# mittinatten/freesasa

Measured on AMD Instinct MI355X. Metric: atoms/sec SASA (L&R 20 slices), higher is better.
Workload: dtype f64

## Files before the change

### freesasa_amd/csrc/engine_internal.h

```cpp
#ifndef FREESASA_AMD_ENGINE_INTERNAL_H
#define FREESASA_AMD_ENGINE_INTERNAL_H

#include <hip/hip_runtime.h>

#include <atomic>
#include <functional>
#include <mutex>
#include <stdint.h>
#include <stddef.h>
#include <stdio.h>
#include <string>
#include <thread>
#include <unistd.h>
#include <vector>

#include "../../include/freesasa_gpu.h"
#include "../../include/freesasa_ingest.h"
#include "sasa_kernels.h"
#include "lr2_kernels.h"
#include "group_kernels.h"
#include "select_kernels.h"
#include "traj_kernels.h"
#include "xtc_kernels.h"
#include "pbc_kernels.h"
#include "pbc_tri_kernels.h"
#include "vol_kernels.h"
#include "dots_kernels.h"
#include "iface_kernels.h"
#include "contact_kernels.h"
#include "rescontact_kernels.h"
#include "ifsweep_kernels.h"
#include "gpu_parse.h"


#define SORT_B 1024
#define SORT_APT 16
#define SORT_ATOMS (SORT_B * SORT_APT - 256)
#define SORT_CELLS (1 << 18)
#define SORT_WORDS (SORT_CELLS / 32)
#define SORT_CELL_BITS 26

hipError_t kl_prep_fused(const sasa::PipeArgs &pa, hipStream_t st);
hipError_t kl_prep_general(const sasa::PipeArgs &pa, long long cells_cap, hipStream_t st);
hipError_t kl_lr2_main(int rmax, int grid, size_t lds, hipStream_t st, const sasa::Lr2Args &la);
hipError_t kl_lr2_mid(int grid, size_t lds, hipStream_t st, const sasa::Lr2Args &la);
hipError_t kl_lr_tile(int tier, const sasa::TileCfg &c, const sasa::TileArgs &t, int grid, size_t lds, hipStream_t st, bool bucket);
hipError_t kl_sr_tile(int tier, const sasa::TileCfg &c, const sasa::TileArgs &t, int grid, size_t lds, hipStream_t st, double *evec = nullptr, unsigned *masks = nullptr);
hipError_t kl_totals(const sasa::PipeArgs &pa, int n_chunks, int n_structs, const double *d_sasa, double *bpart, double *d_totals, hipStream_t st);
hipError_t kl_segment_sums(const double *d_sasa, const int64_t *d_seg, int n_segs, bool short_segments, double *d_out, hipStream_t st);
hipError_t kl_class_sums(const double *d_sasa, const unsigned char *d_class, const int64_t *d_offsets, int n_structs, double *d_out, hipStream_t st);
hipError_t kl_residue_areas(const double *d_sasa, const unsigned char *d_class, const unsigned char *d_backbone, const int64_t *d_res_first,
                            const short *d_ref_row, const double *d_ref_table, double *d_abs, double *d_rel, int n_res, hipStream_t st);
hipError_t kl_arc_kat(const double *d_arcs, const int *d_first, int n_sets, double *d_out, hipStream_t st);
hipError_t kl_widen_f32(const float *d_in, double *d_out, long long n, hipStream_t st);
hipError_t kl_narrow_f64(const double *d_in, float *d_out, long long n, hipStream_t st);
void kl_dump_phase_clocks(void);
hipError_t kl_grp_count(const sasa::GrpArgs &a, hipStream_t st);
hipError_t kl_grp_rank(const sasa::GrpArgs &a, hipStream_t st);
hipError_t kl_grp_finish(const sasa::GrpArgs &a, hipStream_t st);
hipError_t kl_grp_totals(const sasa::GrpArgs &a, hipStream_t st);
hipError_t kl_gid_struct(const sasa::GidArgs &a, hipStream_t st);
hipError_t kl_gid_label(const sasa::GidLabelArgs &a, hipStream_t st);

hipError_t kl_sel_mask(const sasa::SelArgs &a, hipStream_t st);
hipError_t kl_sel_sums(const sasa::SelArgs &a, hipStream_t st);

hipError_t kl_traj_gather(const sasa::TrajArgs &a, const void *d_in, bool in_f32, double *d_out, hipStream_t st);
hipError_t kl_traj_gather_dcd(const sasa::TrajDcdArgs &a, const void *d_in, bool big_endian, double *d_out, hipStream_t st);
hipError_t kl_traj_gather_nc(const sasa::TrajNcArgs &a, const void *d_in, double *d_out, hipStream_t st);
hipError_t kl_traj_gather_trr(const sasa::TrajTrrArgs &a, const void *d_in, bool is_double, double *d_out, hipStream_t st);
hipError_t kl_xtc_scan(const sasa::XtcArgs &a, hipStream_t st);
hipError_t kl_xtc_unpack(const sasa::XtcArgs &a, hipStream_t st);
hipError_t kl_traj_residues(const sasa::TrajArgs &a, hipStream_t st);
hipError_t kl_traj_class(const sasa::TrajArgs &a, hipStream_t st);
hipError_t kl_traj_sel(const sasa::TrajArgs &a, hipStream_t st);
hipError_t kl_traj_group_radii(const sasa::TrajGroupArgs &a, hipStream_t st);
hipError_t kl_traj_group_gather(const sasa::TrajGroupArgs &a, hipStream_t st);
hipError_t kl_traj_group_finish(const sasa::TrajGroupArgs &a, hipStream_t st);
hipError_t kl_traj_group_totals(const sasa::TrajGroupArgs &a, hipStream_t st);
hipError_t kl_traj_stats(const sasa::TrajStatsArgs &a, hipStream_t st);

hipError_t kl_pbc_count(const sasa::PbcArgs &a, hipStream_t st);
hipError_t kl_pbc_emit(const sasa::PbcArgs &a, hipStream_t st);
hipError_t kl_pbc_collect(const sasa::PbcArgs &a, hipStream_t st);
hipError_t kl_pbc_tri_count(const sasa::PbcTriArgs &a, hipStream_t st);
hipError_t kl_pbc_tri_emit(const sasa::PbcTriArgs &a, hipStream_t st);
hipError_t kl_gpbc_cells(const sasa::GpbcArgs &a, hipStream_t st);
hipError_t kl_gpbc_finish(const sasa::GpbcArgs &a, hipStream_t st);

hipError_t kl_vol_origin(const sasa::VolArgs &a, hipStream_t st);
hipError_t kl_vol_atom(const sasa::VolArgs &a, hipStream_t st);

hipError_t kl_dots_count(const sasa::DotsArgs &a, hipStream_t st);
hipError_t kl_dots_expand(const sasa::DotsArgs &a, hipStream_t st);

hipError_t kl_iface_box(const sasa::IfaceArgs &a, hipStream_t st);
hipError_t kl_iface_candidates(const sasa::IfaceArgs &a, hipStream_t st);
hipError_t kl_iface_contact(const sasa::IfaceArgs &a, hipStream_t st);
hipError_t kl_iface_gather(const sasa::IfaceArgs &a, hipStream_t st);
hipError_t kl_iface_finish(const sasa::IfaceArgs &a, hipStream_t st);
hipError_t kl_iface_res_scan(int *a, int64_t n, int *scratch, hipStream_t st);
hipError_t kl_iface_res_segments(const sasa::IfaceResArgs &a, int *scratch, hipStream_t st);
hipError_t kl_iface_res_rows(const sasa::IfaceResArgs &a, int *scratch, hipStream_t st);
hipError_t kl_contact_masks(const sasa::ContactArgs &a, hipStream_t st);
hipError_t kl_contact_attribute(const sasa::ContactArgs &a, hipStream_t st);
hipError_t kl_contact_rows(const sasa::ContactArgs &a, int *scratch, hipStream_t st);
hipError_t kl_rc_segments(const sasa::IfaceResArgs &s, int *scratch, hipStream_t st);
hipError_t kl_rc_fold(const sasa::ResContactArgs &a, int *scratch, hipStream_t st);
hipError_t kl_ifs_side_class(const sasa::IfsClassArgs &a, hipStream_t st);
hipError_t kl_ifs_res_rows(const sasa::IfsRowArgs &a, hipStream_t st);


struct DevBuf {
    void *p = nullptr;
    size_t cap = 0;
};

struct freesasa_gpu_ctx {
    int device = 0;
    hipStream_t stream = nullptr;
    bool own_stream = false;
    bool timing = false;
    bool shared_radii = false;
    char err[512] = {0};
    freesasa_gpu_stats stats = {};
// ... 433 lines not shown
```

### freesasa_amd/csrc/gpu_engine.hip

```cpp
#include <hip/hip_runtime.h>

#include <math.h>
#include <atomic>
#include <new>
#include <stdarg.h>
#include <stdint.h>
#include <stdio.h>
#include <stdlib.h>
#include <string.h>
#include <vector>

#include "engine_internal.h"

using namespace sasa;


int ctx_fail(freesasa_gpu_ctx *c, const char *fmt, ...)
{
    va_list ap;
    va_start(ap, fmt);
    vsnprintf(c->err, sizeof c->err, fmt, ap);
    va_end(ap);
    return -1;
}
// ... 345 lines not shown
{
    c->err[0] = 0;
    if (deferred) *deferred = false;
    if (!d_xyz || !d_radii || !offsets || !d_sasa) return ctx_fail(c, "null argument");
    if (n_structs <= 0) return ctx_fail(c, "n_structs must be > 0");
    if (resolution <= 0) return ctx_fail(c, "resolution must be > 0");
    if (offsets[0] != 0) return ctx_fail(c, "offsets[0] must be 0");
    for (int s = 0; s < n_structs; ++s)
        if (offsets[s + 1] < offsets[s]) return ctx_fail(c, "offsets must be non-decreasing");
    const int64_t n64 = offsets[n_structs];
    if (n64 <= 0) return ctx_fail(c, "empty batch");
    if (n64 > (int64_t)1 << 30) return ctx_fail(c, "batch too large (max 2^30 atoms per call)");
    const int n = (int)n64;

    HIP_TRY(c, hipSetDevice(c->device));
    hipStream_t st = c->stream;
    const size_t nb = (size_t)n;

    if (ensure(c, c->offsets, sizeof(int64_t) * ((size_t)n_structs + 1)) || ensure(c, c->grid, sizeof(GridS) * (size_t)n_structs) ||
        ensure(c, c->ncells, sizeof(long long) * ((size_t)n_structs + 1)) || ensure(c, c->sid, 4 * nb) ||
        ensure(c, c->cell_of, 8 * nb) || ensure(c, c->rank, 4 * nb) || ensure(c, c->sq, 32 * nb) ||
        ensure(c, c->s_idx, 16 * nb) ||
        ensure(c, c->status, sizeof(int) * ST_WORDS))
        return -1;

    if ((int)c->offsets_host.size() != n_structs + 1 ||
        memcmp(c->offsets_host.data(), offsets, sizeof(int64_t) * ((size_t)n_structs + 1)) != 0) {
        if (c->pend[0].active || c->pend[1].active) HIP_TRY(c, hipStreamSynchronize(st));
        c->offsets_host.clear();
        std::vector<int> cs, cl, sc0((size_t)n_structs + 1);
        std::vector<int64_t> cb;
        for (int s = 0; s < n_structs; ++s) {
            sc0[s] = (int)cs.size();
            for (int64_t b = offsets[s]; b < offsets[s + 1]; b += SASA_BOUNDS_CHUNK) {
                const int64_t e = b + SASA_BOUNDS_CHUNK < offsets[s + 1] ? b + SASA_BOUNDS_CHUNK : offsets[s + 1];
                cs.push_back(s); cb.push_back(b); cl.push_back((int)(e - b));
            }
        }
        sc0[n_structs] = (int)cs.size();
        c->n_chunks = (int)cs.size();
        const size_t nc = cs.size();
        if (ensure(c, c->chunk_struct, 4 * nc) || ensure(c, c->chunk_begin, 8 * nc) || ensure(c, c->chunk_len, 4 * nc) ||
            ensure(c, c->struct_chunk0, 4 * ((size_t)n_structs + 1)) || ensure(c, c->bpart, 56 * nc))
            return -1;
        HIP_TRY(c, hipMemcpy(c->offsets.p, offsets, sizeof(int64_t) * ((size_t)n_structs + 1), hipMemcpyHostToDevice));
        HIP_TRY(c, hipMemcpy(c->chunk_struct.p, cs.data(), 4 * nc, hipMemcpyHostToDevice));
        HIP_TRY(c, hipMemcpy(c->chunk_begin.p, cb.data(), 8 * nc, hipMemcpyHostToDevice));
        HIP_TRY(c, hipMemcpy(c->chunk_len.p, cl.data(), 4 * nc, hipMemcpyHostToDevice));
        HIP_TRY(c, hipMemcpy(c->struct_chunk0.p, sc0.data(), 4 * ((size_t)n_structs + 1), hipMemcpyHostToDevice));
        c->offsets_host.assign(offsets, offsets + n_structs + 1);
    }
    HIP_TRY(c, hipMemsetAsync(c->status.p, 0, (sizeof(int) * ST_WORDS + 63) & ~(size_t)63, st));
    if (c->timing) HIP_TRY(c, hipEventRecord(ctx_ev(c)[0], st));

    PipeArgs pa;
    memset(&pa, 0, sizeof pa);
    pa.xyz = d_xyz; pa.radii = d_radii; pa.offsets = (const int64_t *)c->offsets.p;
    pa.n_structs = n_structs; pa.n_atoms = n; pa.probe = probe; pa.max_cells = c->max_cells;
    pa.shared_radii = c->shared_radii ? 1 : 0;
    pa.n_chunks = c->n_chunks; pa.chunk_struct = (const int *)c->chunk_struct.p; pa.chunk_begin = (const int64_t *)c->chunk_begin.p;
    pa.chunk_len = (const int *)c->chunk_len.p; pa.struct_chunk0 = (const int *)c->struct_chunk0.p; pa.bpart = (double *)c->bpart.p;
    pa.grid = (GridS *)c->grid.p; pa.ncells = (long long *)c->ncells.p;
    pa.sid = (int *)c->sid.p; pa.cell_of = (long long *)c->cell_of.p; pa.rank = (int *)c->rank.p;
    pa.sq = (Quad *)c->sq.p;
    pa.s_idx = (SortIdx *)c->s_idx.p;
    pa.status = (int *)c->status.p;
    pa.cells_total = (long long *)((int *)c->status.p + ST_CELLS);
    pa.cells_total_at = pa.cells_total - pa.ncells;
    if (probe != c->hint_probe) {
        c->hint_res[0] = c->hint_res[1] = 0;
        c->hint_pool2 = 0;
        c->hint_probe = probe;
    }
    pa.occ_stride = c->hint_res[lr ? 0 : 1] == resolution ? 0 : (n / 256 > 0 ? n / 256 : 1);

    int *status_h = ctx_status_h(c);
    long long cells_cap = 10LL * n + 256LL * n_structs;
    if (cells_cap < c->cells_hint) cells_cap = c->cells_hint;
    if (cells_cap > c->max_cells) cells_cap = c->max_cells;
    const int nblk_scan = (int)((cells_cap + 1 + (long long)SASA_PIPE_B * SASA_SCAN_ITEMS - 1) / ((long long)SASA_PIPE_B * SASA_SCAN_ITEMS));
    long long biggest = 0;
    for (int s_ = 0; s_ < n_structs; ++s_) biggest = offsets[s_ + 1] - offsets[s_] > biggest ? offsets[s_ + 1] - offsets[s_] : biggest;
    static const long long small_fused = getenv("FREESASA_AMD_SMALL_FUSED") ? atoll(getenv("FREESASA_AMD_SMALL_FUSED")) : 4096;
    const bool fused = c->sort_fused && biggest <= SORT_ATOMS && (n_structs >= 8 || biggest <= small_fused) && !getenv("FREESASA_AMD_NO_FUSED_SORT");
    const bool compact = fused && (!lr || (lr2_supported(resolution) && !getenv("FREESASA_AMD_LR1"))) && !getenv("FREESASA_AMD_DENSE_CELLS");
    if (compact) {
        if (ensure(c, c->cell_tbl, sizeof(unsigned long long) * ((size_t)(cells_cap >> 5) + 2)) || ensure(c, c->cell_first, sizeof(int) * (nb + (size_t)n_structs + 2)))
            return -1;
        pa.cell_tbl = (unsigned long long *)c->cell_tbl.p;
        pa.cell_first = (int *)c->cell_first.p;
    } else {
        const size_t desc_cap_was = c->blk_sums.cap;
        if (ensure(c, c->cell_start, sizeof(int) * ((size_t)cells_cap + 4)) || ensure(c, c->blk_sums, sizeof(unsigned long long) * ((size_t)nblk_scan + 1)))
            return -1;
        if (c->blk_sums.cap != desc_cap_was) HIP_TRY(c, hipMemsetAsync(c->blk_sums.p, 0, c->blk_sums.cap, st));
    }
    pa.cell_start = (int *)c->cell_start.p;
    pa.scan_desc = (unsigned long long *)c->blk_sums.p;
    c->scan_epoch = c->scan_epoch >= (1 << 30) - 1 ? 1 : c->scan_epoch + 1;
    pa.scan_epoch = c->scan_epoch;
    pa.zero_n = cells_cap + 2;
    pa.cells_cap = cells_cap;

    if (fused) {
        HIP_TRY(c, kl_prep_fused(pa, st));
    } else {
        HIP_TRY(c, kl_prep_general(pa, cells_cap, st));
    }
    if (c->timing) HIP_TRY(c, hipEventRecord(ctx_ev(c)[1], st));

    if (lr && lr2_supported(resolution) && !getenv("FREESASA_AMD_LR1")) {
        const int rc2 = run_lr2(c, pa, n, n_structs, resolution, d_sasa, d_totals, defer && !c->dbg_nn);
        if (rc2 == 0 && defer && !c->dbg_nn && deferred) *deferred = true;
        return rc2;
    }

    const int hi = lr ? 0 : 1;
    if (c->hint_res[hi] != resolution) {
        long long total_cells = 0;
        const int rcs = collect_status(c, n_structs, 8, &total_cells);
        if (rcs) return rcs;
        if (status_h[ST_OCC_N] > 0) {
            const double nn_est = 3.1 * (double)status_h[ST_OCC_SUM] / (double)status_h[ST_OCC_N];
            const TileCfg probe_cfg = choose_cfg(resolution, lr, 0, !lr && resolution <= SR_CAP_POINTS_MAX);
            int pool = (int)(1.35 * nn_est * probe_cfg.TA + 16.0);
            pool = (pool + 1) & ~1;
            if (pool < 32) pool = 32;
            if (pool > 4096) pool = 4096;
            if (!lr) {
                pool = (((int)(1.5 * nn_est) + 8 + 7) / 8) * 8;
                pool = pool < SR_CAP_MIN ? SR_CAP_MIN : (pool > SR_CAP_MAX ? SR_CAP_MAX : pool);
            }
            c->hint_res[hi] = resolution;
            c->hint_ta[hi] = probe_cfg.TA;
            c->hint_pool[hi] = pool;
            if (lr) c->hint_bucket = nn_est > 30.0;
        }
    }
    if (!lr) {
        if (!unit_points) return ctx_fail(c, "unit_points is null");
        if (ensure(c, c->unit_pts, sizeof(double) * 3 * (size_t)resolution)) return -1;
        if (c->unit_host.size() != 3 * (size_t)resolution ||
            memcmp(c->unit_host.data(), unit_points, sizeof(double) * 3 * (size_t)resolution) != 0) {
            c->unit_host.assign(unit_points, unit_points + 3 * (size_t)resolution);
            if (hipMemcpyAsync(c->unit_pts.p, c->unit_host.data(), sizeof(double) * 3 * (size_t)resolution, hipMemcpyHostToDevice, st) != hipSuccess) {
                c->unit_host.clear();
                return ctx_fail(c, "upload of the test points failed");
            }
            int tn = SR_CAP_N_DEFAULT, tl = SR_CAP_L_DEFAULT;
            if (const char *e = getenv("FREESASA_AMD_SR_CAPS")) {
                int n_ = 0, l_ = 0;
                if (sscanf(e, "%d,%d", &n_, &l_) == 2 && n_ >= 1 && n_ <= 64 && l_ >= 1 && l_ <= 256) { tn = n_; tl = l_; }
                else if (atoi(e) == 0) tn = 0;
            }
            c->captab_n = c->captab_l = 0;
            bool built = false;
            try { built = tn > 0 && sr_captab_build(c->unit_host.data(), resolution, tn, tl, c->captab_host); }
            catch (...) { c->unit_host.clear(); throw; }
            if (built) {
                const size_t bytes = sizeof(SrCapEntry) * c->captab_host.size();
                if (ensure(c, c->captab, bytes)) { c->unit_host.clear(); return -1; }
                if (hipMemcpyAsync(c->captab.p, c->captab_host.data(), bytes, hipMemcpyHostToDevice, st) != hipSuccess) {
                    c->unit_host.clear();
                    return ctx_fail(c, "upload of the cap table failed");
                }
                c->captab_n = tn; c->captab_l = tl;
            }
        }
    }

    const bool sr_caps = !lr && c->captab_n > 0;
    double *const evec = lr ? nullptr : c->vol_evec;
    unsigned *const masks = lr ? nullptr : c->sr_masks;
    if (evec && masks) return ctx_fail(c, "the exposure masks and the volume's vectors cannot be asked for in one batch: one store phase makes one of them");
    const char *const what = masks ? "the exposure masks" : "the volume", *const is = masks ? "are" : "is", *const needs = masks ? "need" : "needs";
    if ((evec || masks) && !sr_caps) {
        if (resolution > SR_CAP_POINTS_MAX) return ctx_fail(c, "%s %s offered up to %d test points (%d asked for)", what, is, SR_CAP_POINTS_MAX, resolution);
        const char *e = getenv("FREESASA_AMD_SR_CAPS");
        if (e && atoi(e) == 0 && !strchr(e, ',')) return ctx_fail(c, "%s %s the cap-mask kernel, which FREESASA_AMD_SR_CAPS=0 switches off", what, needs);
        return ctx_fail(c, "%s %s unit test points: these are not unit vectors", what, needs);
    }
    TileCfg cfg = choose_cfg(resolution, lr, c->hint_res[hi] == resolution ? c->hint_pool[hi] : 0, sr_caps, c->hint_res[hi] == resolution ? c->hint_ta[hi] : 0);
    if (const char *e = getenv("FREESASA_AMD_CFG")) {
        int b = 0, t = 0, pl = 0, d = 0;
        if (sscanf(e, "%d,%d,%d,%d", &b, &t, &pl, &d) == 4 && (b == 64 || b == 128 || b == 256) && t >= 1 && t <= b &&
            (!lr || !cfg.tab || t * resolution <= 4096)) {
            cfg.B = b; cfg.TA = t; cfg.pool = pl; cfg.ds = lr ? d : 0;
            if (!lr) { cfg.cap_idx = pl > 0 ? pl : cfg.cap_idx; cfg.pool = cfg.TA * cfg.cap_idx; }
// ... 221 lines not shown
```

### freesasa_amd/csrc/gpu_kernels.hip

```cpp
#include <hip/hip_runtime.h>

#include <math.h>
#include <mutex>
#include <stdint.h>
#include <stdio.h>
#include <stdlib.h>
#include <string.h>

#include "sasa_kernels.h"
#ifdef SASA_PHASE_TIMING
__device__ unsigned long long g_phase_clock[16];
#define LR2_MARK_BEGIN unsigned long long lr2_last_ = wall_clock64(); if (lane == 0 && !a.work_items && ((p0 / a.TA) & 255) == 0) atomicAdd(&g_phase_clock[15], 1ULL)
#define LR2_MARK(k) do { if (lane == 0 && !a.work_items && ((p0 / a.TA) & 255) == 0) { const unsigned long long now_ = wall_clock64(); \
        atomicAdd(&g_phase_clock[(k)], now_ - lr2_last_); lr2_last_ = now_; } } while (0)
#endif
#include "engine_internal.h"

using namespace sasa;


__global__ __launch_bounds__(SASA_PIPE_B) void k_prep_general(PipeArgs a)
{
    __shared__ double red[7 * SASA_PIPE_B], red2[7 * 16];
    __shared__ int last;
    {
        const Int4 z = {0, 0, 0, 0};
        const long long words = a.zero_n >> 2;
        for (long long w = (long long)blockIdx.x * SASA_PIPE_B + threadIdx.x; w < words; w += (long long)gridDim.x * SASA_PIPE_B)
            ((Int4 *)a.cell_start)[w] = z;
        if (blockIdx.x == 0 && threadIdx.x < (a.zero_n & 3)) a.cell_start[(words << 2) + threadIdx.x] = 0;
    }
    if ((int)blockIdx.x < a.n_chunks) {
        bounds_phase0(a, red, blockIdx.x, threadIdx.x, SASA_PIPE_B);
        __syncthreads();
        bounds_phase1(red, red2, threadIdx.x, SASA_PIPE_B);
        __syncthreads();
        bounds_phase2(a, red2, blockIdx.x, threadIdx.x);
    }
    __threadfence();
    __syncthreads();
    if (threadIdx.x == 0) last = atomicAdd(&a.status[ST_TICKET_PREP], 1) == (int)gridDim.x - 1;
    __syncthreads();
    if (!last) return;
    __threadfence();
    for (int s0 = 0; s0 < a.n_structs; s0 += SASA_PIPE_B / SASA_GRID_GROUP) {
        __syncthreads();
        grid_phase0(a, red, s0, threadIdx.x);
        __syncthreads();
        grid_phase1(a, red, s0, threadIdx.x);
    }
    __syncthreads();
    long long *part = (long long *)red, *part2 = (long long *)red2;
    cellbase_phase0(a, part, threadIdx.x, SASA_PIPE_B);
    __syncthreads();
    cellbase_phase1(part, part2, threadIdx.x, SASA_PIPE_B);
    __syncthreads();
    cellbase_phase1b(a, part2, threadIdx.x);
    __syncthreads();
    cellbase_phase2(a, part, part2, threadIdx.x, SASA_PIPE_B);
}

#define PIPE_GATE(st) do { if ((st)[ST_ERROR] | (st)[ST_RETRY]) return; } while (0)

__global__ __launch_bounds__(SASA_PIPE_B) void k_count(PipeArgs a)
{
    __shared__ int cells[SASA_PIPE_B], base[SASA_PIPE_B];
    PIPE_GATE(a.status);
    const int i = blockIdx.x * SASA_PIPE_B + threadIdx.x;
    count_phase0(a, cells, i, threadIdx.x);
    __syncthreads();
    count_phase1(a, cells, base, threadIdx.x, SASA_PIPE_B);
    __syncthreads();
    count_phase2(a, cells, base, i, threadIdx.x);
}

static_assert(SASA_PIPE_B == SASA_SCAN_GROUP * SASA_SCAN_GROUP, "two-level combine of the scan partials");
__device__ __forceinline__ int scan_blocks(long long n)
{
    return (int)((n + 1 + (long long)SASA_PIPE_B * SASA_SCAN_ITEMS - 1) / ((long long)SASA_PIPE_B * SASA_SCAN_ITEMS));
}
__global__ __launch_bounds__(SASA_PIPE_B) void k_scan(PipeArgs a)
{
    __shared__ int part[SASA_PIPE_B], part2[SASA_SCAN_GROUP], blk_s, before;
    ScanRegs r;
    PIPE_GATE(a.status);
    const long long n = *cell_total(a);
    if (threadIdx.x == 0) blk_s = scan_take_block(a);
    __syncthreads();
    const int blk = blk_s;
    if (blk >= scan_blocks(n)) return;
    scan_phase0(a, n, part, blk, threadIdx.x, SASA_PIPE_B, r);
    __syncthreads();
    scan_phase1(part, part2, threadIdx.x);
    __syncthreads();
    scan_phase2(a, part2, &before, blk, threadIdx.x);
    __syncthreads();
    scan_phase3(a, n, part, part2, &before, blk, threadIdx.x, SASA_PIPE_B, r);
}

__global__ __launch_bounds__(SASA_PIPE_B) void k_scatter(PipeArgs a)
{
    PIPE_GATE(a.status);
    scatter_atom(a, blockIdx.x * SASA_PIPE_B + threadIdx.x);
}

__device__ __forceinline__ int sort_block_scan(int v, int *scratch, int tid)
{
    const int lane = tid & 63, wave = tid >> 6;
    int incl = v;
    for (int d = 1; d < 64; d <<= 1) {
        const int o = __shfl_up(incl, d, 64);
        if (lane >= d) incl += o;
    }
    __syncthreads();
    if (lane == 63) scratch[wave] = incl;
    __syncthreads();
    if (tid < 64) {
        const int w = tid < SORT_B / 64 ? scratch[tid] : 0;
        int wi = w;
        for (int d = 1; d < SORT_B / 64; d <<= 1) {
            const int o = __shfl_up(wi, d, 64);
            if (tid >= d) wi += o;
        }
        if (tid < SORT_B / 64) scratch[tid] = wi - w;
        if (tid == SORT_B / 64 - 1) scratch[SORT_B / 64] = wi;
    }
    __syncthreads();
    return scratch[wave] + incl - v;
}
__global__ __launch_bounds__(SORT_B) void k_sort_struct(PipeArgs a)
{
    __shared__ unsigned bm[SORT_WORDS];
    __shared__ unsigned short wpre[SORT_WORDS];
    __shared__ unsigned cnt[SORT_ATOMS / 2 + 2];
    __shared__ int scratch[SORT_B / 64 + 1];
    double (*const red)[SORT_B / 64] = (double (*)[SORT_B / 64])wpre;
    __shared__ GridS g_sh;
    __shared__ long long c_sh;
    const int s = blockIdx.x, tid = threadIdx.x;
    const long long b0 = a.offsets[s];
    const int n = (int)(a.offsets[s + 1] - b0);
    if (n <= 0) {
        if (tid == 0) { GridS e; e.x0 = e.y0 = e.z0 = 0; e.d = 1; e.nx = e.ny = e.nz = 0; e.cell_base = 0; a.grid[s] = e; a.ncells[s] = 0; }
        return;
    }
    if (n > SORT_ATOMS) {
        if (tid == 0) atomicOr(&a.status[ST_RETRY], 2);
        return;
    }
    {
        double lo0 = INFINITY, lo1 = INFINITY, lo2 = INFINITY, hi0 = -INFINITY, hi1 = -INFINITY, hi2 = -INFINITY, rmax = 0;
        int bad = 0;
        for (int li = tid; li < n; li += SORT_B) {
            const long long i = b0 + li;
            const double x = a.xyz[3 * i], y = a.xyz[3 * i + 1], z = a.xyz[3 * i + 2];
            lo0 = fmin(x, lo0); hi0 = fmax(x, hi0);
            lo1 = fmin(y, lo1); hi1 = fmax(y, hi1);
            lo2 = fmin(z, lo2); hi2 = fmax(z, hi2);
            const double rr = a.radii[a.shared_radii ? (long long)li : i];
            rmax = fmax(rr + a.probe, rmax);
            if (!(x - x == 0) || !(y - y == 0) || !(z - z == 0)) bad = ERR_BAD_COORD;
            if (!(rr - rr == 0)) bad = bad ? bad : ERR_BAD_RADIUS;
        }
        if (bad) atomicMax(&a.status[ST_ERROR], bad);
        for (int d = 1; d < 64; d <<= 1) {
            lo0 = fmin(lo0, __shfl_xor(lo0, d, 64)); lo1 = fmin(lo1, __shfl_xor(lo1, d, 64)); lo2 = fmin(lo2, __shfl_xor(lo2, d, 64));
            hi0 = fmax(hi0, __shfl_xor(hi0, d, 64)); hi1 = fmax(hi1, __shfl_xor(hi1, d, 64)); hi2 = fmax(hi2, __shfl_xor(hi2, d, 64));
            rmax = fmax(rmax, __shfl_xor(rmax, d, 64));
        }
        if ((tid & 63) == 0) {
            const int w = tid >> 6;
            red[0][w] = lo0; red[1][w] = lo1; red[2][w] = lo2; red[3][w] = hi0; red[4][w] = hi1; red[5][w] = hi2; red[6][w] = rmax;
        }
        __syncthreads();
        if (tid == 0) {
            double lo[3] = {INFINITY, INFINITY, INFINITY}, hi[3] = {-INFINITY, -INFINITY, -INFINITY}, rm = 0;
            for (int w = 0; w < SORT_B / 64; ++w) {
                for (int k = 0; k < 3; ++k) { lo[k] = fmin(red[k][w], lo[k]); hi[k] = fmax(red[3 + k][w], hi[k]); }
                rm = fmax(red[6][w], rm);
            }
            GridS g;
            const double d = 2 * rm;
            int err = ERR_NONE;
            if (!(d > 0) || !(d < INFINITY)) err = ERR_BAD_RADIUS;
            for (int k = 0; k < 3; ++k)
                if (!(lo[k] > -INFINITY && hi[k] < INFINITY)) err = err ? err : ERR_BAD_COORD;
            long long nc = 0;
            g.d = d;
            g.x0 = lo[0] - d / 2.; g.y0 = lo[1] - d / 2.; g.z0 = lo[2] - d / 2.;
            g.nx = g.ny = g.nz = 0; g.cell_base = 0;
            if (!err) {
                const double fx = ceil((hi[0] + d / 2. - g.x0) / d);
                const double fy = ceil((hi[1] + d / 2. - g.y0) / d);
                const double fz = ceil((hi[2] + d / 2. - g.z0) / d);
                if (!(fx * fy * fz <= (double)a.max_cells) || !(fx >= 1 && fy >= 1 && fz >= 1)) err = ERR_GRID_TOO_BIG;
                else { g.nx = (int)fx; g.ny = (int)fy; g.nz = (int)fz; nc = (long long)g.nx * g.ny * g.nz; }
            }
            if (err) {
                atomicMax(&a.status[ST_ERROR], err);
                g.nx = g.ny = g.nz = 1; g.d = 1; g.x0 = g.y0 = g.z0 = 0;
                nc = 1;
            }
            const long long take = a.cell_tbl ? ((nc + 1 + 31) & ~31LL) : nc + 1;
            const long long base = (long long)atomicAdd((unsigned long long *)&a.ncells[a.cells_total_at], (unsigned long long)take);
            if (base + nc + 1 > a.max_cells) { atomicMax(&a.status[ST_ERROR], (int)ERR_GRID_TOO_BIG); nc = -1; }
            else if (nc > (1LL << SORT_CELL_BITS)) { atomicOr(&a.status[ST_RETRY], 2); nc = -1; }
            else if (a.cells_cap > 0 && base + nc + 1 > a.cells_cap) { atomicOr(&a.status[ST_RETRY], 1); nc = -1; }
            else if (a.status[ST_RETRY] | a.status[ST_ERROR]) nc = -1;
            g.cell_base = (int)base;
            a.grid[s] = g;
            a.ncells[s] = nc < 0 ? 0 : nc;
            g_sh = g; c_sh = nc;
        }
        __syncthreads();
    }
    const GridS g = g_sh;
    if (c_sh < 0) return;
    const int C = (int)c_sh;
    unsigned cellf[SORT_APT];
    for (int k = 0; k < SORT_APT; ++k) {
        const int li = tid + k * SORT_B;
        cellf[k] = 0xffffffffu;
        if (li < n) {
            const long long i = b0 + li;
            int ix = cell_coord(a.xyz[3 * i], g.x0, g.d);
            int iy = cell_coord(a.xyz[3 * i + 1], g.y0, g.d);
            int iz = cell_coord(a.xyz[3 * i + 2], g.z0, g.d);
            if (!(ix >= 0 && ix < g.nx && iy >= 0 && iy < g.ny && iz >= 0 && iz < g.nz)) {
                if (a.status[ST_ERROR] == 0) atomicMax(&a.status[ST_ERROR], (int)ERR_BAD_COORD);
                ix = iy = iz = 0;
            }
            const int c = ix + g.nx * (iy + g.ny * iz);
            const int fl = (ix == 0 ? CELL_X0 : 0) | (ix == g.nx - 1 ? CELL_X1 : 0) | (iy == 0 ? CELL_Y0 : 0) |
                           (iy == g.ny - 1 ? CELL_Y1 : 0) | (iz == 0 ? CELL_Z0 : 0) | (iz == g.nz - 1 ? CELL_Z1 : 0);
            cellf[k] = (unsigned)c | ((unsigned)fl << SORT_CELL_BITS);
        }
        if ((k & 3) == 3) __asm__ volatile("" ::: "memory");
    }
    const unsigned cmask = (1u << SORT_CELL_BITS) - 1u;
    int base = 0;
    int occ_done = 0;
    const long long occ_base = b0 + s;
    for (int lo = 0; lo < C; lo += SORT_CELLS) {
        const int Cp = C - lo < SORT_CELLS ? C - lo : SORT_CELLS, W = (Cp + 31) >> 5;
        __syncthreads();
        for (int w = tid; w < W; w += SORT_B) bm[w] = 0;
        for (int k = tid; k < n / 2 + 2; k += SORT_B) cnt[k] = 0;
        __syncthreads();
        for (int k = 0; k < SORT_APT; ++k) {
            const int cc = (int)(cellf[k] & cmask) - lo;
            if (cellf[k] != 0xffffffffu && cc >= 0 && cc < Cp) atomicOr(&bm[cc >> 5], 1u << (cc & 31));
        }
        __syncthreads();
        {
            int pc[SORT_WORDS / SORT_B], sum = 0;
            for (int j = 0; j < SORT_WORDS / SORT_B; ++j) {
                const int w = tid * (SORT_WORDS / SORT_B) + j;
                pc[j] = w < W ? __popc(bm[w]) : 0;
                sum += pc[j];
            }
            int run = sort_block_scan(sum, scratch, tid);
            for (int j = 0; j < SORT_WORDS / SORT_B; ++j) {
                const int w = tid * (SORT_WORDS / SORT_B) + j;
                if (w < W) wpre[w] = (unsigned short)run;
                run += pc[j];
            }
        }
        __syncthreads();
        const int occ = scratch[SORT_B / 64];
        unsigned place[SORT_APT];
        for (int k = 0; k < SORT_APT; ++k) {
            place[k] = 0xffffffffu;
            const int cc = (int)(cellf[k] & cmask) - lo;
            if (cellf[k] != 0xffffffffu && cc >= 0 && cc < Cp) {
                const int oc = (int)wpre[cc >> 5] + __popc(bm[cc >> 5] & ((1u << (cc & 31)) - 1u));
                const unsigned old = atomicAdd(&cnt[oc >> 1], (oc & 1) ? 0x10000u : 1u);
                place[k] = (unsigned)oc | (((old >> ((oc & 1) * 16)) & 0xffffu) << 16);
            }
        }
        __syncthreads();
        unsigned short *const c16 = (unsigned short *)cnt;
        {
            int v[SORT_APT], sum = 0;
            for (int j = 0; j < SORT_APT; ++j) {
                const int e = tid * SORT_APT + j;
                v[j] = e < occ ? (int)c16[e] : 0;
                sum += v[j];
            }
            int run = sort_block_scan(sum, scratch, tid);
            for (int j = 0; j < SORT_APT; ++j) {
                const int e = tid * SORT_APT + j;
                if (e <= occ) c16[e] = (unsigned short)run;
                run += v[j];
            }
        }
        __syncthreads();
        const int n_pass = scratch[SORT_B / 64];
        for (int k = 0; k < SORT_APT; ++k) {
            if (place[k] == 0xffffffffu) continue;
            const int li = tid + k * SORT_B;
            const long long i = b0 + li;
            const int oc = (int)(place[k] & 0xffffu);
            const long long p = b0 + base + c16[oc] + (int)(place[k] >> 16);
            Quad v;
            v.x = a.xyz[3 * i]; v.y = a.xyz[3 * i + 1]; v.z = a.xyz[3 * i + 2];
            v.w = a.radii[a.shared_radii ? (long long)li : i] + a.probe;
            a.sq[p] = v;
            SortIdx si;
            si.cell = (long long)((unsigned long long)(unsigned)(g.cell_base + (int)(cellf[k] & cmask)) |
                                  ((unsigned long long)((cellf[k] >> SORT_CELL_BITS) | cell_pack_grid(g.nx, g.ny)) << 32));
            si.orig = (int)i; si.strct = s;
            a.s_idx[p] = si;
            if (a.occ_stride > 0 && i % a.occ_stride == 0) {
                atomicAdd(&a.status[ST_OCC_SUM], (int)c16[oc + 1] - (int)c16[oc]);
                atomicAdd(&a.status[ST_OCC_N], 1);
            }
            if ((k & 3) == 3) __asm__ volatile("" ::: "memory");
        }
        if (a.cell_tbl) {
            unsigned long long *const tbl = a.cell_tbl + (((long long)g.cell_base + lo) >> 5);
            for (int w = tid; w < W; w += SORT_B) tbl[w] = (unsigned long long)bm[w] | ((unsigned long long)(unsigned)(occ_base + occ_done + wpre[w]) << 32);
            for (int e = tid; e < occ; e += SORT_B) a.cell_first[occ_base + occ_done + e] = (int)(b0 + base + c16[e]);
        } else {
            for (int cc = tid; cc < Cp; cc += SORT_B) {
                const int oc = (int)wpre[cc >> 5] + __popc(bm[cc >> 5] & ((1u << (cc & 31)) - 1u));
                a.cell_start[g.cell_base + lo + cc] = (int)(b0 + base + c16[oc]);
            }
        }
        base += n_pass;
        occ_done += occ;
    }
    if (tid == 0) {
        if (a.cell_tbl) {
            a.cell_first[occ_base + occ_done] = (int)(b0 + n);
            if ((C & 31) == 0) a.cell_tbl[((long long)g.cell_base + C) >> 5] = (unsigned long long)(unsigned)(occ_base + occ_done) << 32;
        } else {
            a.cell_start[g.cell_base + C] = (int)(b0 + n);
        }
    }
}

__global__ __launch_bounds__(SASA_TOT_B) void k_totals(const double *sasa, const int64_t *offsets, int n_structs, double *totals)
{
    __shared__ double part[SASA_TOT_B];
    totals_phase0(sasa, offsets, part, blockIdx.x, threadIdx.x);
    __syncthreads();
    totals_phase1(part, totals, blockIdx.x, threadIdx.x);
}

__global__ __launch_bounds__(SASA_TOT_B) void k_totals_chunks(PipeArgs a, const double *sasa, double *chunk_tot)
{
    __shared__ double part[SASA_TOT_B];
    totals_chunk_phase0(a, sasa, part, blockIdx.x, threadIdx.x);
    __syncthreads();
    totals_chunk_phase1(part, chunk_tot, blockIdx.x, threadIdx.x);
}
__global__ __launch_bounds__(256) void k_totals_structs(PipeArgs a, const double *chunk_tot, double *totals)
{
    totals_struct(a, chunk_tot, totals, blockIdx.x * 256 + threadIdx.x);
}

__global__ __launch_bounds__(256) void k_segsum_small(const double *sasa, const int64_t *seg, int n_segs, double *out)
{
    segsum_small(sasa, seg, out, blockIdx.x * 256 + threadIdx.x, n_segs);
}

__global__ __launch_bounds__(256) void k_residue_areas(const double *sasa, const unsigned char *cls, const unsigned char *bb,
                                                      const int64_t *res_first, const short *ref_row, const double *ref_table,
                                                      double *abs_out, double *rel_out, int n_res)
{
    residue_areas(sasa, cls, bb, res_first, ref_row, ref_table, abs_out, rel_out, blockIdx.x * 256 + threadIdx.x, n_res);
}

__global__ __launch_bounds__(SASA_TOT_B) void k_class_sums(const double *sasa, const unsigned char *cls, const int64_t *offsets, double *out)
{
    __shared__ double part[3 * SASA_TOT_B];
    class_phase0(sasa, cls, offsets, part, blockIdx.x, threadIdx.x);
    __syncthreads();
    class_phase1(part, out, blockIdx.x, threadIdx.x);
}

#ifdef SASA_PHASE_TIMING
#define PHASE_MARK(k) do { if (tid == 0 && TIER == 0 && (tile & 255) == 0) { const unsigned long long now_ = wall_clock64(); \
        atomicAdd(&g_phase_clock[k], now_ - last_); last_ = now_; } } while (0)
#else
#define PHASE_MARK(k) do { } while (0)
#endif
template <int B, bool GLOBAL, int TIER, int WPE, bool BUCKET = false>
__global__ __launch_bounds__(B) __attribute__((amdgpu_waves_per_eu(WPE, WPE))) void k_lr_tile(TileArgs a, int items)
{
    extern __shared__ __attribute__((aligned(16))) char smem[];
    const int tid = threadIdx.x;
    PIPE_GATE(a.status);
    TileMem m = tile_carve<GLOBAL>(a, smem, items, B, blockIdx.x);
    const int n_work = a.work_tiles ? *a.work_count : ((a.n_tiles + 7) >> 3) << 3;
    int wg_max_nn = 0;
    for (int w = blockIdx.x; w < n_work; w += gridDim.x) {
        const int tile = a.work_tiles ? a.work_tiles[w] : xcd_tile(w, a.n_tiles);
        if (tile >= a.n_tiles) continue;
#ifdef SASA_PHASE_TIMING
        unsigned long long last_ = wall_clock64();
#endif
        tile_phase_load(a, m, tile, tid, B, BUCKET);
        __syncthreads();
        PHASE_MARK(0);
        tile_phase_neighbors(a, m, tile, tid, B);
        __syncthreads();
// ... 229 lines not shown
        }
    } else return hipErrorInvalidValue;
    return hipGetLastError();
}
template <bool GLOBAL, int TIER>
static hipError_t launch_sr(const TileCfg &c, const TileArgs &t, int grid, size_t lds, hipStream_t s, double *evec, unsigned *masks)
{
    if constexpr (!GLOBAL) {
        if (sr_caps_shape(c, t, false)) {
            if (evec) {
                if (c.B == 256)
                    hipLaunchKernelGGL((k_sr_tile_vol<256, TIER>), dim3(grid), dim3(256), lds, s, t, c.items, evec);
                else if (c.B == 128)
                    hipLaunchKernelGGL((k_sr_tile_vol<128, TIER>), dim3(grid), dim3(128), lds, s, t, c.items, evec);
                else if (c.B == 64)
                    hipLaunchKernelGGL((k_sr_tile_vol<64, TIER>), dim3(grid), dim3(64), lds, s, t, c.items, evec);
                else return hipErrorInvalidValue;
                return hipGetLastError();
            }
            if (masks) {
                if (c.B == 256)
                    hipLaunchKernelGGL((k_sr_tile_mask<256, TIER>), dim3(grid), dim3(256), lds, s, t, c.items, masks);
                else if (c.B == 128)
                    hipLaunchKernelGGL((k_sr_tile_mask<128, TIER>), dim3(grid), dim3(128), lds, s, t, c.items, masks);
                else if (c.B == 64)
                    hipLaunchKernelGGL((k_sr_tile_mask<64, TIER>), dim3(grid), dim3(64), lds, s, t, c.items, masks);
                else return hipErrorInvalidValue;
                return hipGetLastError();
            }
            if (c.B == 256)
                hipLaunchKernelGGL((k_sr_tile<256, false, TIER, true>), dim3(grid), dim3(256), lds, s, t, c.items);
            else if (c.B == 128)
                hipLaunchKernelGGL((k_sr_tile<128, false, TIER, true>), dim3(grid), dim3(128), lds, s, t, c.items);
            else if (c.B == 64)
                hipLaunchKernelGGL((k_sr_tile<64, false, TIER, true>), dim3(grid), dim3(64), lds, s, t, c.items);
            else return hipErrorInvalidValue;
            return hipGetLastError();
        }
    }
    if (c.B == 256)
        hipLaunchKernelGGL((k_sr_tile<256, GLOBAL, TIER>), dim3(grid), dim3(256), lds, s, t, c.items);
    else if (c.B == 128)
        hipLaunchKernelGGL((k_sr_tile<128, GLOBAL, TIER>), dim3(grid), dim3(128), lds, s, t, c.items);
    else if (c.B == 64)
        hipLaunchKernelGGL((k_sr_tile<64, GLOBAL, TIER>), dim3(grid), dim3(64), lds, s, t, c.items);
    else return hipErrorInvalidValue;
    return hipGetLastError();
}

static void allow_large_lds()
{
    static std::once_flag attr_once;
    std::call_once(attr_once, [] {
        const void *fns[] = {(const void *)k_lr_tile<256, false, 0, 4>, (const void *)k_lr_tile<128, false, 0, 4>, (const void *)k_lr_tile<64, false, 0, 4>,
                             (const void *)k_lr_tile<256, false, 1, 4>, (const void *)k_lr_tile<128, false, 1, 4>, (const void *)k_lr_tile<64, false, 1, 4>,
                             (const void *)k_lr_tile<64, false, 0, 4, true>, (const void *)k_lr_tile<64, false, 1, 4, true>,
                             (const void *)k_sr_tile<256, false, 0>, (const void *)k_sr_tile<128, false, 0>, (const void *)k_sr_tile<64, false, 0>,
                             (const void *)k_sr_tile<256, false, 1>, (const void *)k_sr_tile<128, false, 1>, (const void *)k_sr_tile<64, false, 1>,
                             (const void *)k_sr_tile<256, false, 0, true>, (const void *)k_sr_tile<128, false, 0, true>, (const void *)k_sr_tile<64, false, 0, true>,
                             (const void *)k_sr_tile<256, false, 1, true>, (const void *)k_sr_tile<128, false, 1, true>, (const void *)k_sr_tile<64, false, 1, true>,
                             (const void *)k_sr_tile_vol<256, 0>, (const void *)k_sr_tile_vol<128, 0>, (const void *)k_sr_tile_vol<64, 0>,
                             (const void *)k_sr_tile_vol<256, 1>, (const void *)k_sr_tile_vol<128, 1>, (const void *)k_sr_tile_vol<64, 1>,
                             (const void *)k_sr_tile_mask<256, 0>, (const void *)k_sr_tile_mask<128, 0>, (const void *)k_sr_tile_mask<64, 0>,
                             (const void *)k_sr_tile_mask<256, 1>, (const void *)k_sr_tile_mask<128, 1>, (const void *)k_sr_tile_mask<64, 1>};
        for (const void *fn : fns) (void)hipFuncSetAttribute(fn, hipFuncAttributeMaxDynamicSharedMemorySize, 160 * 1024);
    });
}

hipError_t kl_lr_tile(int tier, const TileCfg &c, const TileArgs &t, int grid, size_t lds, hipStream_t st, bool bucket)
{
    allow_large_lds();
    if (tier == 0) return launch_lr<false, 0>(c, t, grid, lds, st, bucket);
    if (tier == 1) return launch_lr<false, 1>(c, t, grid, lds, st, bucket);
    return launch_lr<true, 2>(c, t, grid, lds, st, false);
}
hipError_t kl_sr_tile(int tier, const TileCfg &c, const TileArgs &t, int grid, size_t lds, hipStream_t st, double *evec, unsigned *masks)
{
    allow_large_lds();
    if (tier == 0) return launch_sr<false, 0>(c, t, grid, lds, st, evec, masks);
    if (tier == 1) return launch_sr<false, 1>(c, t, grid, lds, st, evec, masks);
    return launch_sr<true, 2>(c, t, grid, lds, st, nullptr, nullptr);
}

hipError_t kl_prep_fused(const PipeArgs &pa, hipStream_t st)
{
    hipLaunchKernelGGL(k_sort_struct, dim3(pa.n_structs), dim3(SORT_B), 0, st, pa);
    return hipGetLastError();
}
hipError_t kl_prep_general(const PipeArgs &pa, long long cells_cap, hipStream_t st)
{
    const int nblk_scan = (int)((cells_cap + 1 + (long long)SASA_PIPE_B * SASA_SCAN_ITEMS - 1) / ((long long)SASA_PIPE_B * SASA_SCAN_ITEMS));
    const int nblk_atoms = (pa.n_atoms + SASA_PIPE_B - 1) / SASA_PIPE_B;
    long long zb = (pa.zero_n * 4 + 65535) / 65536;
    if (zb > 2048) zb = 2048;
    hipLaunchKernelGGL(k_prep_general, dim3((unsigned)(pa.n_chunks + zb)), dim3(SASA_PIPE_B), 0, st, pa);
    hipLaunchKernelGGL(k_count, dim3(nblk_atoms), dim3(SASA_PIPE_B), 0, st, pa);
    hipLaunchKernelGGL(k_scan, dim3(nblk_scan), dim3(SASA_PIPE_B), 0, st, pa);
    hipLaunchKernelGGL(k_scatter, dim3(nblk_atoms), dim3(SASA_PIPE_B), 0, st, pa);
    return hipGetLastError();
}

hipError_t kl_totals(const PipeArgs &pa, int n_chunks, int n_structs, const double *d_sasa, double *bpart, double *d_totals, hipStream_t st)
{
    hipLaunchKernelGGL(k_totals_chunks, dim3(n_chunks), dim3(SASA_TOT_B), 0, st, pa, d_sasa, bpart);
    hipLaunchKernelGGL(k_totals_structs, dim3((n_structs + 255) / 256), dim3(256), 0, st, pa, (const double *)bpart, d_totals);
    return hipGetLastError();
}

__global__ __launch_bounds__(SASA_TOT_B) void k_vol_origin(VolArgs a)
{
    __shared__ double part[6 * SASA_TOT_B];
    vol_origin_phase0(a, part, blockIdx.x, threadIdx.x);
    __syncthreads();
    vol_origin_phase1(a, part, blockIdx.x, threadIdx.x);
}
__global__ __launch_bounds__(VOL_B) void k_vol_atom(VolArgs a)
{
    vol_atom(a, (int64_t)blockIdx.x * VOL_B + threadIdx.x);
}
hipError_t kl_vol_origin(const VolArgs &a, hipStream_t st)
{
    hipLaunchKernelGGL(k_vol_origin, dim3((unsigned)a.n_structs), dim3(SASA_TOT_B), 0, st, a);
    return hipGetLastError();
}
hipError_t kl_vol_atom(const VolArgs &a, hipStream_t st)
{
    hipLaunchKernelGGL(k_vol_atom, dim3((unsigned)((a.n_atoms + VOL_B - 1) / VOL_B)), dim3(VOL_B), 0, st, a);
    return hipGetLastError();
}

__global__ __launch_bounds__(DOTS_SCAN_T) void k_dots_block_sums(DotsArgs a)
{
    __shared__ int part[DOTS_SCAN_T];
    dots_count_phase0(a, part, blockIdx.x, threadIdx.x);
    __syncthreads();
    dots_count_phase1(a, part, blockIdx.x, threadIdx.x);
}
__global__ __launch_bounds__(DOTS_SCAN_T) void k_dots_scan_blocks(DotsArgs a)
{
    __shared__ int64_t part[DOTS_SCAN_T];
    dots_scan_phase0(a, part, threadIdx.x);
    __syncthreads();
    dots_scan_phase1(a, part, threadIdx.x);
    __syncthreads();
    dots_scan_phase2(a, part, threadIdx.x);
}
__global__ __launch_bounds__(DOTS_SCAN_T) void k_dots_first(DotsArgs a)
{
    __shared__ int part[DOTS_SCAN_T];
    dots_first_phase0(a, part, blockIdx.x, threadIdx.x);
    __syncthreads();
    dots_first_phase1(a, part, blockIdx.x, threadIdx.x);
    __syncthreads();
    dots_first_phase2(a, part, blockIdx.x, threadIdx.x);
}
__global__ __launch_bounds__(DOTS_EXPAND_B) void k_dots_expand(DotsArgs a)
{
    dots_expand(a, (int64_t)blockIdx.x, threadIdx.x);
}
hipError_t kl_dots_count(const DotsArgs &a, hipStream_t st)
{
    hipLaunchKernelGGL(k_dots_block_sums, dim3((unsigned)a.n_blocks), dim3(DOTS_SCAN_T), 0, st, a);
    hipLaunchKernelGGL(k_dots_scan_blocks, dim3(1), dim3(DOTS_SCAN_T), 0, st, a);
    hipLaunchKernelGGL(k_dots_first, dim3((unsigned)a.n_blocks), dim3(DOTS_SCAN_T), 0, st, a);
    return hipGetLastError();
}
hipError_t kl_dots_expand(const DotsArgs &a, hipStream_t st)
{
    const int64_t pairs = a.n_atoms * a.n_points;
    const int64_t per_wg = (int64_t)DOTS_EXPAND_B * DOTS_EXPAND_U;
// ... 614 lines not shown
```

Before: 1.104 billion.

## Templatize fused sort kernel on shape and keep coordinates in registers/LDS

Makes the per-structure sort kernel a template over block size, atoms per thread, cell table size and a KEEP flag, and picks a shape from a table based on the largest structure. With KEEP, x/y coordinates stay in registers and z in shared memory, so the kernel does not re-read xyz from global memory in the cell-assignment and scatter passes. Waves-per-EU hints and asm barriers are added to steer register allocation. The cost is more registers and LDS per block, which can lower occupancy, and more template instantiations.

```diff
diff --git a/freesasa_amd/csrc/engine_internal.h b/freesasa_amd/csrc/engine_internal.h
--- a/freesasa_amd/csrc/engine_internal.h
+++ b/freesasa_amd/csrc/engine_internal.h
@@ -18,6 +18,7 @@
 #include "../../include/freesasa_ingest.h"
 #include "sasa_kernels.h"
 #include "lr2_kernels.h"
+#include "sort_shapes.h"
 #include "group_kernels.h"
 #include "select_kernels.h"
 #include "traj_kernels.h"
@@ -33,14 +34,8 @@
 #include "gpu_parse.h"
 
 
-#define SORT_B 1024
-#define SORT_APT 16
-#define SORT_ATOMS (SORT_B * SORT_APT - 256)
-#define SORT_CELLS (1 << 18)
-#define SORT_WORDS (SORT_CELLS / 32)
-#define SORT_CELL_BITS 26
-
-hipError_t kl_prep_fused(const sasa::PipeArgs &pa, hipStream_t st);
+
+hipError_t kl_prep_fused(const sasa::PipeArgs &pa, int shape, hipStream_t st);
 hipError_t kl_prep_general(const sasa::PipeArgs &pa, long long cells_cap, hipStream_t st);
 hipError_t kl_lr2_main(int rmax, int grid, size_t lds, hipStream_t st, const sasa::Lr2Args &la);
 hipError_t kl_lr2_mid(int grid, size_t lds, hipStream_t st, const sasa::Lr2Args &la);
diff --git a/freesasa_amd/csrc/gpu_engine.hip b/freesasa_amd/csrc/gpu_engine.hip
--- a/freesasa_amd/csrc/gpu_engine.hip
+++ b/freesasa_amd/csrc/gpu_engine.hip
@@ -451,7 +451,10 @@
     long long biggest = 0;
     for (int s_ = 0; s_ < n_structs; ++s_) biggest = offsets[s_ + 1] - offsets[s_] > biggest ? offsets[s_ + 1] - offsets[s_] : biggest;
     static const long long small_fused = getenv("FREESASA_AMD_SMALL_FUSED") ? atoll(getenv("FREESASA_AMD_SMALL_FUSED")) : 4096;
-    const bool fused = c->sort_fused && biggest <= SORT_ATOMS && (n_structs >= 8 || biggest <= small_fused) && !getenv("FREESASA_AMD_NO_FUSED_SORT");
+    int sort_b = 0, sort_apt = 0;
+    if (const char *e = getenv("FREESASA_AMD_SORT")) (void)sscanf(e, "%d,%d", &sort_b, &sort_apt);
+    const int sort_shape = sort_choose_shape(biggest, sort_b, sort_apt);
+    const bool fused = c->sort_fused && sort_shape >= 0 && (n_structs >= 8 || biggest <= small_fused) && !getenv("FREESASA_AMD_NO_FUSED_SORT");
     const bool compact = fused && (!lr || (lr2_supported(resolution) && !getenv("FREESASA_AMD_LR1"))) && !getenv("FREESASA_AMD_DENSE_CELLS");
     if (compact) {
         if (ensure(c, c->cell_tbl, sizeof(unsigned long long) * ((size_t)(cells_cap >> 5) + 2)) || ensure(c, c->cell_first, sizeof(int) * (nb + (size_t)n_structs + 2)))
@@ -471,8 +474,12 @@
     pa.zero_n = cells_cap + 2;
     pa.cells_cap = cells_cap;
 
+    if (getenv("FREESASA_AMD_SHOW_SHAPE")) {
+        if (fused) fprintf(stderr, "sort shape: B %d apt %d cells 2^%d keep %d (largest structure %lld)\n", sort_shapes[sort_shape].B, sort_shapes[sort_shape].apt, sort_shapes[sort_shape].log_cells, sort_shapes[sort_shape].keep, biggest);
+        else fprintf(stderr, "sort shape: general pipeline (largest structure %lld)\n", biggest);
+    }
     if (fused) {
-        HIP_TRY(c, kl_prep_fused(pa, st));
+        HIP_TRY(c, kl_prep_fused(pa, sort_shape, st));
     } else {
         HIP_TRY(c, kl_prep_general(pa, cells_cap, st));
     }
diff --git a/freesasa_amd/csrc/gpu_kernels.hip b/freesasa_amd/csrc/gpu_kernels.hip
--- a/freesasa_amd/csrc/gpu_kernels.hip
+++ b/freesasa_amd/csrc/gpu_kernels.hip
@@ -104,6 +104,7 @@
     scatter_atom(a, blockIdx.x * SASA_PIPE_B + threadIdx.x);
 }
 
+template <int SORT_B>
 __device__ __forceinline__ int sort_block_scan(int v, int *scratch, int tid)
 {
     const int lane = tid & 63, wave = tid >> 6;
@@ -128,12 +129,19 @@
     __syncthreads();
     return scratch[wave] + incl - v;
 }
-__global__ __launch_bounds__(SORT_B) void k_sort_struct(PipeArgs a)
-{
+template <int SORT_B, int SORT_APT, int LOGC, int KEEP, int WPE>
+__global__ __launch_bounds__(SORT_B) __attribute__((amdgpu_waves_per_eu(WPE, WPE))) void k_sort_struct(PipeArgs a)
+{
+    constexpr int SORT_CELLS = 1 << LOGC;
+    constexpr int SORT_WORDS = SORT_CELLS / 32;
+    constexpr int SORT_ATOMS = sort_shape_atoms(SORT_B, SORT_APT);
+    static_assert(SORT_ATOMS < SORT_B * SORT_APT && SORT_ATOMS < 65536 && SORT_WORDS % SORT_B == 0 && SORT_B % 64 == 0 && SORT_B / 64 <= 64, "k_sort_struct shape");
+    static_assert(7 * (SORT_B / 64) * sizeof(double) <= SORT_WORDS * sizeof(unsigned short), "the bounds' partials lie in wpre");
     __shared__ unsigned bm[SORT_WORDS];
     __shared__ unsigned short wpre[SORT_WORDS];
     __shared__ unsigned cnt[SORT_ATOMS / 2 + 2];
     __shared__ int scratch[SORT_B / 64 + 1];
+    __shared__ double zs[KEEP ? SORT_ATOMS : 1];
     double (*const red)[SORT_B / 64] = (double (*)[SORT_B / 64])wpre;
     __shared__ GridS g_sh;
     __shared__ long long c_sh;
@@ -148,9 +156,31 @@
         if (tid == 0) atomicOr(&a.status[ST_RETRY], 2);
         return;
     }
+    double px[KEEP ? SORT_APT : 1], py[KEEP ? SORT_APT : 1];
     {
         double lo0 = INFINITY, lo1 = INFINITY, lo2 = INFINITY, hi0 = -INFINITY, hi1 = -INFINITY, hi2 = -INFINITY, rmax = 0;
         int bad = 0;
+        if constexpr (KEEP != 0) {
+#pragma unroll
+            for (int k = 0; k < SORT_APT; ++k) {
+                const int li = tid + k * SORT_B < n ? tid + k * SORT_B : n - 1;
+                const long long i = b0 + li;
+                px[k] = a.xyz[3 * i]; py[k] = a.xyz[3 * i + 1];
+            }
+#pragma unroll
+            for (int k = 0; k < SORT_APT; ++k) {
+                const int li = tid + k * SORT_B < n ? tid + k * SORT_B : n - 1;
+                const double x = px[k], y = py[k], z = a.xyz[3 * (b0 + li) + 2];
+                if (tid + k * SORT_B < n) zs[li] = z;
+                lo0 = fmin(x, lo0); hi0 = fmax(x, hi0);
+                lo1 = fmin(y, lo1); hi1 = fmax(y, hi1);
+                lo2 = fmin(z, lo2); hi2 = fmax(z, hi2);
+                const double rr = a.radii[a.shared_radii ? (long long)li : b0 + li];
+                rmax = fmax(rr + a.probe, rmax);
+                if (!(x - x == 0) || !(y - y == 0) || !(z - z == 0)) bad = ERR_BAD_COORD;
+                if (!(rr - rr == 0)) bad = bad ? bad : ERR_BAD_RADIUS;
+            }
+        } else
         for (int li = tid; li < n; li += SORT_B) {
             const long long i = b0 + li;
             const double x = a.xyz[3 * i], y = a.xyz[3 * i + 1], z = a.xyz[3 * i + 2];
@@ -221,11 +251,11 @@
     for (int k = 0; k < SORT_APT; ++k) {
         const int li = tid + k * SORT_B;
         cellf[k] = 0xffffffffu;
-        if (li < n) {
+        if (KEEP || li < n) {
             const long long i = b0 + li;
-            int ix = cell_coord(a.xyz[3 * i], g.x0, g.d);
-            int iy = cell_coord(a.xyz[3 * i + 1], g.y0, g.d);
-            int iz = cell_coord(a.xyz[3 * i + 2], g.z0, g.d);
+            int ix = cell_coord(KEEP ? px[k] : a.xyz[3 * i], g.x0, g.d);
+            int iy = cell_coord(KEEP ? py[k] : a.xyz[3 * i + 1], g.y0, g.d);
+            int iz = cell_coord(KEEP ? zs[li < n ? li : n - 1] : a.xyz[3 * i + 2], g.z0, g.d);
             if (!(ix >= 0 && ix < g.nx && iy >= 0 && iy < g.ny && iz >= 0 && iz < g.nz)) {
                 if (a.status[ST_ERROR] == 0) atomicMax(&a.status[ST_ERROR], (int)ERR_BAD_COORD);
                 ix = iy = iz = 0;
@@ -233,7 +263,7 @@
             const int c = ix + g.nx * (iy + g.ny * iz);
             const int fl = (ix == 0 ? CELL_X0 : 0) | (ix == g.nx - 1 ? CELL_X1 : 0) | (iy == 0 ? CELL_Y0 : 0) |
                            (iy == g.ny - 1 ? CELL_Y1 : 0) | (iz == 0 ? CELL_Z0 : 0) | (iz == g.nz - 1 ? CELL_Z1 : 0);
-            cellf[k] = (unsigned)c | ((unsigned)fl << SORT_CELL_BITS);
+            cellf[k] = li < n ? (unsigned)c | ((unsigned)fl << SORT_CELL_BITS) : 0xffffffffu;
         }
         if ((k & 3) == 3) __asm__ volatile("" ::: "memory");
     }
@@ -243,9 +273,12 @@
     const long long occ_base = b0 + s;
     for (int lo = 0; lo < C; lo += SORT_CELLS) {
         const int Cp = C - lo < SORT_CELLS ? C - lo : SORT_CELLS, W = (Cp + 31) >> 5;
-        __syncthreads();
-        for (int w = tid; w < W; w += SORT_B) bm[w] = 0;
-        for (int k = tid; k < n / 2 + 2; k += SORT_B) cnt[k] = 0;
+        int tl = tid;
+        __asm__ volatile("" : "+v"(tl));
+        for (int k = 0; k < SORT_APT; ++k) __asm__ volatile("" : "+v"(cellf[k]));
+        __syncthreads();
+        for (int w = tl; w < W; w += SORT_B) bm[w] = 0;
+        for (int k = tl; k < n / 2 + 2; k += SORT_B) cnt[k] = 0;
         __syncthreads();
         for (int k = 0; k < SORT_APT; ++k) {
             const int cc = (int)(cellf[k] & cmask) - lo;
@@ -255,13 +288,13 @@
         {
             int pc[SORT_WORDS / SORT_B], sum = 0;
             for (int j = 0; j < SORT_WORDS / SORT_B; ++j) {
-                const int w = tid * (SORT_WORDS / SORT_B) + j;
+                const int w = tl * (SORT_WORDS / SORT_B) + j;
                 pc[j] = w < W ? __popc(bm[w]) : 0;
                 sum += pc[j];
             }
-            int run = sort_block_scan(sum, scratch, tid);
+            int run = sort_block_scan<SORT_B>(sum, scratch, tl);
             for (int j = 0; j < SORT_WORDS / SORT_B; ++j) {
-                const int w = tid * (SORT_WORDS / SORT_B) + j;
+                const int w = tl * (SORT_WORDS / SORT_B) + j;
                 if (w < W) wpre[w] = (unsigned short)run;
                 run += pc[j];
             }
@@ -283,13 +316,13 @@
         {
             int v[SORT_APT], sum = 0;
             for (int j = 0; j < SORT_APT; ++j) {
-                const int e = tid * SORT_APT + j;
+                const int e = tl * SORT_APT + j;
                 v[j] = e < occ ? (int)c16[e] : 0;
                 sum += v[j];
             }
-            int run = sort_block_scan(sum, scratch, tid);
+            int run = sort_block_scan<SORT_B>(sum, scratch, tl);
             for (int j = 0; j < SORT_APT; ++j) {
-                const int e = tid * SORT_APT + j;
+                const int e = tl * SORT_APT + j;
                 if (e <= occ) c16[e] = (unsigned short)run;
                 run += v[j];
             }
@@ -298,12 +331,12 @@
         const int n_pass = scratch[SORT_B / 64];
         for (int k = 0; k < SORT_APT; ++k) {
             if (place[k] == 0xffffffffu) continue;
-            const int li = tid + k * SORT_B;
+            const int li = tl + k * SORT_B;
             const long long i = b0 + li;
             const int oc = (int)(place[k] & 0xffffu);
             const long long p = b0 + base + c16[oc] + (int)(place[k] >> 16);
             Quad v;
-            v.x = a.xyz[3 * i]; v.y = a.xyz[3 * i + 1]; v.z = a.xyz[3 * i + 2];
+            v.x = KEEP ? px[k] : a.xyz[3 * i]; v.y = KEEP ? py[k] : a.xyz[3 * i + 1]; v.z = KEEP ? zs[li] : a.xyz[3 * i + 2];
             v.w = a.radii[a.shared_radii ? (long long)li : i] + a.probe;
             a.sq[p] = v;
             SortIdx si;
@@ -311,7 +344,7 @@
                                   ((unsigned long long)((cellf[k] >> SORT_CELL_BITS) | cell_pack_grid(g.nx, g.ny)) << 32));
             si.orig = (int)i; si.strct = s;
             a.s_idx[p] = si;
-            if (a.occ_stride > 0 && i % a.occ_stride == 0) {
+            if (a.occ_stride > 0 && (unsigned)i % (unsigned)a.occ_stride == 0) {
                 atomicAdd(&a.status[ST_OCC_SUM], (int)c16[oc + 1] - (int)c16[oc]);
                 atomicAdd(&a.status[ST_OCC_N], 1);
             }
@@ -319,10 +352,10 @@
         }
         if (a.cell_tbl) {
             unsigned long long *const tbl = a.cell_tbl + (((long long)g.cell_base + lo) >> 5);
-            for (int w = tid; w < W; w += SORT_B) tbl[w] = (unsigned long long)bm[w] | ((unsigned long long)(unsigned)(occ_base + occ_done + wpre[w]) << 32);
-            for (int e = tid; e < occ; e += SORT_B) a.cell_first[occ_base + occ_done + e] = (int)(b0 + base + c16[e]);
+            for (int w = tl; w < W; w += SORT_B) tbl[w] = (unsigned long long)bm[w] | ((unsigned long long)(unsigned)(occ_base + occ_done + wpre[w]) << 32);
+            for (int e = tl; e < occ; e += SORT_B) a.cell_first[occ_base + occ_done + e] = (int)(b0 + base + c16[e]);
         } else {
-            for (int cc = tid; cc < Cp; cc += SORT_B) {
+            for (int cc = tl; cc < Cp; cc += SORT_B) {
                 const int oc = (int)wpre[cc >> 5] + __popc(bm[cc >> 5] & ((1u << (cc & 31)) - 1u));
                 a.cell_start[g.cell_base + lo + cc] = (int)(b0 + base + c16[oc]);
             }
@@ -718,10 +751,21 @@
     return launch_sr<true, 2>(c, t, grid, lds, st, nullptr, nullptr);
 }
 
-hipError_t kl_prep_fused(const PipeArgs &pa, hipStream_t st)
-{
-    hipLaunchKernelGGL(k_sort_struct, dim3(pa.n_structs), dim3(SORT_B), 0, st, pa);
-    return hipGetLastError();
+template <int K>
+static hipError_t launch_sort(const PipeArgs &pa, hipStream_t st)
+{
+    constexpr SortShape s = sort_shapes[K];
+    hipLaunchKernelGGL((k_sort_struct<s.B, s.apt, s.log_cells, s.keep, s.resident * s.B / 256>), dim3(pa.n_structs), dim3(s.B), 0, st, pa);
+    return hipGetLastError();
+}
+hipError_t kl_prep_fused(const PipeArgs &pa, int shape, hipStream_t st)
+{
+    static_assert(SORT_N_SHAPES == 2, "one case per shape");
+    switch (shape) {
+    case 0: return launch_sort<0>(pa, st);
+    case 1: return launch_sort<1>(pa, st);
+    default: return hipErrorInvalidValue;
+    }
 }
 hipError_t kl_prep_general(const PipeArgs &pa, long long cells_cap, hipStream_t st)
 {
diff --git a/freesasa_amd/csrc/sort_shapes.h b/freesasa_amd/csrc/sort_shapes.h
--- /dev/null
+++ b/freesasa_amd/csrc/sort_shapes.h
@@ -0,0 +1,39 @@
+#ifndef FREESASA_AMD_SORT_SHAPES_H
+#define FREESASA_AMD_SORT_SHAPES_H
+
+namespace sasa {
+
+struct SortShape {
+    int B, apt, log_cells, keep, resident;
+    int atoms;
+    int from;
+};
+
+#define SORT_CELL_BITS 26
+
+constexpr int sort_shape_atoms(int B, int apt) { return B * apt == 16384 ? 16384 - 256 : B * apt - 1; }
+
+#define SORT_N_SHAPES 2
+static constexpr SortShape sort_shapes[SORT_N_SHAPES] = {
+    {1024, 10, 18, 1, 1, sort_shape_atoms(1024, 10), 7681},
+    {1024, 16, 18, 0, 1, sort_shape_atoms(1024, 16), 0},
+};
+
+constexpr long long sort_shape_table_bytes(const SortShape &s)
+{
+    return (1LL << s.log_cells) / 32 * 4 + (1LL << s.log_cells) / 32 * 2 + ((long long)s.atoms / 2 + 2) * 4 + (s.keep ? 8LL * s.atoms : 0);
+}
+
+static inline int sort_choose_shape(long long biggest, int force_b = 0, int force_apt = 0)
+{
+    if (force_b > 0 && force_apt > 0)
+        for (int k = 0; k < SORT_N_SHAPES; ++k)
+            if (sort_shapes[k].B == force_b && sort_shapes[k].apt == force_apt && biggest <= sort_shapes[k].atoms) return k;
+    for (int k = 0; k < SORT_N_SHAPES; ++k)
+        if (biggest >= sort_shapes[k].from && biggest <= sort_shapes[k].atoms) return k;
+    return -1;
+}
+
+}
+
+#endif
```

Result: no change. 1.108 billion (median of 6 runs) (+0.3%).
